# dwcoen1234/longfellow-zk

Hardware: AMD Instinct MI355X
Metric: FFT field-elems/s (batched FFT 2^20 x 1024 rows, Fp128) (higher is better)
Workload: dtype u128 (Fp128 Montgomery, 4 x u32 limbs); 1 GPU; batched FFT 2^20 points x 1024 rows per GPU, Fp128 fftb, in place in HBM; field=Fp128 p=2^128-2^108+1, rows_per_gpu=1024, n=1048576, parallelism=rows sharded x1

## Files before the change

longfellow-zk_amd/csrc/fft.hip:

```cpp
#include <string>
#include <type_traits>

#include "ctx.h"
#include "fp_tile_arith.h"

int lf_lch14_fft_bitsliced(lfgpu_ctx* c, int k, int inverse, size_t rows, unsigned l, u64 coset, void* d_B, size_t ld);

#define TILE_ELTS 8192u

struct TilePlan {
  const elt_t* src;
  elt_t* dst;
  long long src_row, dst_row;
  long long src_tile, dst_tile;
  long long sk, sc, dk, dc;
  u32 logT, logC, nbatch;
  u32 kfast_src, kfast_dst;
  u32 wlds;
};

__device__ __forceinline__ u32 bitrev(u32 x, u32 bits) { return bits ? (__brev(x) >> (32 - bits)) : 0; }

__device__ __forceinline__ u32 lds_slot(u32 k, u32 c, u32 logT, u32 logC) {
  u32 slot = (k << logC) + c;
  if (logT >= 8 && logC >= 3) slot ^= (k >> (logT - 4)) & 15u;
  return slot;
}

struct Fp128Ops {
  static constexpr const char* kKey = "fp";
  static LF_HD elt_t add(elt_t a, elt_t b) { return fp_add(a, b); }
  static LF_HD elt_t sub(elt_t a, elt_t b) { return fp_sub(a, b); }
  static LF_HD elt_t mul_tw(elt_t a, elt_t w) { return fp_mul(a, w); }
  static elt_t hmul(elt_t a, elt_t b) { return fp_mul(a, b); }
  static elt_t one() { return h_fp_of_scalar(1); }
  static elt_t inv(elt_t a) { return h_fp_inv(a); }
};
static u64 h_f64_pow(u64 x, u64 e) {
  u64 r = 0xFFFFFFFFull;
  for (; e; e >>= 1) {
    if (e & 1) r = f64_mul(r, x);
    x = f64_mul(x, x);
  }
  return r;
}
template <bool REAL>
struct F64x2Ops {
  static constexpr const char* kKey = "f64x2";
  static LF_HD elt_t add(elt_t a, elt_t b) { return f64x2_add(a, b); }
  static LF_HD elt_t sub(elt_t a, elt_t b) { return f64x2_sub(a, b); }
  static LF_HD elt_t mul_tw(elt_t a, elt_t w) { return REAL ? f64x2_mul_real(a, w.lo) : f64x2_mul(a, w); }
  static elt_t hmul(elt_t a, elt_t b) { return f64x2_mul(a, b); }
  static elt_t one() { return elt_t{0xFFFFFFFFull, 0ull}; }
  static elt_t inv(elt_t a) {
    const u64 d = f64_add(f64_mul(a.lo, a.lo), f64_mul(a.hi, a.hi));
    return f64x2_mul_real(elt_t{a.lo, f64_sub(0, a.hi)}, h_f64_pow(d, F64_P - 2));
  }
};

template <class O, int R, int FFT_THREADS>
__device__ __forceinline__ void fp_radix_round(elt_t* s, const elt_t* Wl, u32 wsh, u32 logT, u32 logC, u32 st, u32 tid) {
  constexpr u32 N = 1u << R;
  const u32 T = 1u << logT, C = 1u << logC, m = 1u << st;
  for (u32 e = tid; e < (T >> R) * C; e += FFT_THREADS) {
    const u32 c = e & (C - 1), b = e >> logC;
    const u32 j = b & (m - 1);
    const u32 i0 = ((b >> st) << (st + R)) + j;
    elt_t x[N];
    u32 q[N];
#pragma unroll
    for (u32 a = 0; a < N; ++a) {
      q[a] = lds_slot(i0 + a * m, c, logT, logC);
      x[a] = ld16(&s[q[a]]);
    }
#pragma unroll
    for (u32 t = 0; t < (u32)R; ++t) {
      const u32 half = 1u << t;
#pragma unroll
      for (u32 a = 0; a < N; ++a) {
        if (a & half) continue;
        const u32 jj = j + (a & (half - 1)) * m;
        if (t > 0 || j) {
          if ((a & (half - 1)) || j) x[a + half] = O::mul_tw(x[a + half], ld16(&Wl[(size_t)(jj << (logT - 1 - st - t)) << wsh]));
        }
        const elt_t u = x[a], v = x[a + half];
        x[a] = O::add(u, v);
        x[a + half] = O::sub(u, v);
      }
    }
#pragma unroll
    for (u32 a = 0; a < N; ++a) st16(&s[q[a]], x[a]);
  }
}

template <class O, int FFT_THREADS, bool WLDS>
__global__ __launch_bounds__(FFT_THREADS) void fp_fft_tile(TilePlan p, const elt_t* __restrict__ W, u32 wshift,
                                                           const elt_t* __restrict__ tw_lo,
                                                           const elt_t* __restrict__ tw_hi, u32 row_fast) {
  extern __shared__ elt_t s[];
  const u32 T = 1u << p.logT, C = 1u << p.logC, tid = threadIdx.x;
  const u32 bx = row_fast ? blockIdx.y : blockIdx.x, by = row_fast ? blockIdx.x : blockIdx.y;
  const u32 cbase = bx << p.logC;
  const elt_t* src = p.src + (long long)by * p.src_row + (long long)bx * p.src_tile;
  elt_t* dst = p.dst + (long long)by * p.dst_row + (long long)bx * p.dst_tile;

  for (u32 e = tid; e < T * C; e += FFT_THREADS) {
    u32 k, c;
    if (p.kfast_src) { k = e & (T - 1); c = e >> p.logT; } else { c = e & (C - 1); k = e >> p.logC; }
    elt_t v = elt_zero();
    if (cbase + c < p.nbatch) v = ld16(src + (long long)k * p.sk + (long long)c * p.sc);
    st16(&s[lds_slot(bitrev(k, p.logT), c, p.logT, p.logC)], v);
  }
  elt_t* const wl = s + (T << p.logC);
  if (WLDS)
    for (u32 i = tid; i < (T >> 1); i += FFT_THREADS) st16(&wl[i], ld16(&W[(size_t)i << wshift]));
  const u32 wsh = WLDS ? 0 : wshift;
  __syncthreads();
  u32 st = 0;
  while (st < p.logT) {
    const u32 rem = p.logT - st;
    const u32 R = (rem == 3 || rem > 4) ? 3 : (rem >= 2 ? 2 : 1);
    if (WLDS) {
      if (R == 3) fp_radix_round<O, 3, FFT_THREADS>(s, wl, wsh, p.logT, p.logC, st, tid);
      else if (R == 2) fp_radix_round<O, 2, FFT_THREADS>(s, wl, wsh, p.logT, p.logC, st, tid);
      else fp_radix_round<O, 1, FFT_THREADS>(s, wl, wsh, p.logT, p.logC, st, tid);
    } else {
      if (R == 3) fp_radix_round<O, 3, FFT_THREADS>(s, W, wsh, p.logT, p.logC, st, tid);
      else if (R == 2) fp_radix_round<O, 2, FFT_THREADS>(s, W, wsh, p.logT, p.logC, st, tid);
      else fp_radix_round<O, 1, FFT_THREADS>(s, W, wsh, p.logT, p.logC, st, tid);
    }
    __syncthreads();
    st += R;
  }
  for (u32 e = tid; e < T * C; e += FFT_THREADS) {
    u32 j, c;
    if (p.kfast_dst) { j = e & (T - 1); c = e >> p.logT; } else { c = e & (C - 1); j = e >> p.logC; }
    if (cbase + c >= p.nbatch) continue;
    elt_t v = ld16(&s[lds_slot(j, c, p.logT, p.logC)]);
    if (tw_lo) {
      const u32 col = cbase + c, ex = j * col;
      if (ex) {
        if (tw_hi) {
          elt_t t = ld16(&tw_lo[ex & 1023]);
          if (ex >> 10) t = O::mul_tw(t, ld16(&tw_hi[ex >> 10]));
          v = O::mul_tw(v, t);
        } else {
          v = O::mul_tw(v, ld16(&tw_lo[(size_t)j * p.nbatch + col]));
        }
      }
    }
    st16(dst + (long long)j * p.dk + (long long)c * p.dc, v);
  }
}

template <class O>
struct T4Ops : O {
  static __device__ __forceinline__ elt_t add_lazy(elt_t a, elt_t b) { return O::add(a, b); }
  static __device__ __forceinline__ elt_t canon(elt_t a) { return a; }
};
#if defined(__HIP_DEVICE_COMPILE__)
template <>
struct T4Ops<Fp128Ops> : Fp128Ops {
  static __device__ __forceinline__ elt_t add(elt_t a, elt_t b) { return fpt_add(a, b); }
  static __device__ __forceinline__ elt_t add_lazy(elt_t a, elt_t b) { return fpt_add_lazy(a, b); }
  static __device__ __forceinline__ elt_t canon(elt_t a) { return fpt_canon(a); }
  static __device__ __forceinline__ elt_t sub(elt_t a, elt_t b) { return fpt_sub(a, b); }
  static __device__ __forceinline__ elt_t mul_tw(elt_t a, elt_t w) { return fpt_mul(a, w); }
};
#endif

__device__ __forceinline__ u32 t4_slot(u32 p, u32 c, u32 p7) { return ((p << 2) | c) ^ p7; }
__device__ __forceinline__ u32 t4_wslot(u32 i) { return i ^ ((i >> 4) & 15u); }

enum : u32 { T4_CANON = 0, T4_LAZY = 1, T4_LAZY_OUT = 2 };
template <class O, u32 ST, u32 R, bool ROUND0, u32 LZ = T4_CANON>
__device__ __forceinline__ void t4_stages(elt_t* x, u32 j, const elt_t* wl, const elt_t* __restrict__ W, u32 wshift) {
#pragma unroll
  for (u32 t = 0; t < R; ++t) {
    const u32 half = 1u << t;
#pragma unroll
    for (u32 a = 0; a < (1u << R); ++a) {
      if (a & half) continue;
      const u32 jj = j + (a & (half - 1)) * (1u << ST), sh = 9 - ST - t;
      if (!ROUND0) x[a + half] = T4Ops<O>::mul_tw(x[a + half], ld16(&wl[t4_wslot(jj << sh)]));
      else if (a & (half - 1)) x[a + half] = T4Ops<O>::mul_tw(x[a + half], ld16(&W[(size_t)(jj << sh) << wshift]));
      const bool last = LZ == T4_LAZY_OUT && t == R - 1;
      const bool full = LZ == T4_CANON || last || (ROUND0 && ((t == 0 && a != 0) || (t == 1 && a == 4)));
      const elt_t u = last ? T4Ops<O>::canon(x[a]) : x[a], v = x[a + half];
      x[a] = full ? T4Ops<O>::add(u, v) : T4Ops<O>::add_lazy(u, v);
      x[a + half] = T4Ops<O>::sub(u, v);
    }
  }
}

template <class O, u32 LZ>
__device__ __forceinline__ void t4_round0(elt_t* s, const elt_t* y, u32 kb, u32 c, const elt_t* wl, const elt_t* __restrict__ W, u32 wshift) {
  elt_t x[8];
#pragma unroll
  for (u32 a = 0; a < 8; ++a) x[a] = y[((a & 1) << 2) | (a & 2) | (a >> 2)];
  t4_stages<O, 0, 3, true, LZ>(x, 0, wl, W, wshift);
  const u32 b = __brev(kb) >> 25, s0 = t4_slot(8 * b, c, b >> 4), s1 = t4_slot(8 * b + 1, c, b >> 4);
#pragma unroll
  for (u32 a = 0; a < 8; a += 2) {
    st16(&s[s0 + 4 * a], x[a]);
    st16(&s[s1 + 4 * a], x[a + 1]);
  }
}
template <class O, u32 LZ>
__device__ __forceinline__ void t4_round1(elt_t* s, u32 tid, const elt_t* wl, const elt_t* __restrict__ W, u32 wshift) {
  const u32 c = tid & 3, j = (tid >> 2) & 7, h = tid >> 5;
  const u32 s0 = t4_slot(64 * h + j, c, h >> 1);
  elt_t x[8];
#pragma unroll
  for (u32 a = 0; a < 8; ++a) x[a] = ld16(&s[s0 + 32 * a]);
  t4_stages<O, 3, 3, false, LZ>(x, j, wl, W, wshift);
#pragma unroll
  for (u32 a = 0; a < 8; ++a) st16(&s[s0 + 32 * a], x[a]);
}
__device__ __forceinline__ u32 t4_round2_load(elt_t* x, const elt_t* s, u32 e) {
  const u32 c = e & 3, h = e >> 8, j = (e >> 2) & 63;
  const u32 s0 = t4_slot(256 * h + j, c, 2 * h);
#pragma unroll
  for (u32 a = 0; a < 4; ++a) x[a] = ld16(&s[(s0 ^ (a >> 1)) + 256 * a]);
  return s0;
}
template <class O, u32 LZ>
__device__ __forceinline__ void t4_round2_finish(elt_t* s, elt_t* x, u32 e, u32 s0, const elt_t* wl, const elt_t* __restrict__ W, u32 wshift) {
  t4_stages<O, 6, 2, false, LZ>(x, (e >> 2) & 63, wl, W, wshift);
#pragma unroll
  for (u32 a = 0; a < 4; ++a) st16(&s[(s0 ^ (a >> 1)) + 256 * a], x[a]);
}
template <class O, u32 LZ>
__device__ __forceinline__ void t4_round2(elt_t* s, u32 e, const elt_t* wl, const elt_t* __restrict__ W, u32 wshift) {
  elt_t x[4];
  const u32 s0 = t4_round2_load(x, s, e);
  t4_round2_finish<O, LZ>(s, x, e, s0, wl, W, wshift);
}
__device__ __forceinline__ void t4_round3_load(elt_t* x, const elt_t* s, u32 e) {
  const u32 c = e & 3, j = e >> 2;
  const u32 s0 = t4_slot(j, c, j >> 7);
#pragma unroll
  for (u32 a = 0; a < 4; ++a) x[a] = ld16(&s[(s0 ^ (2 * a)) + 1024 * a]);
}

__device__ __forceinline__ void t4_xcd_order(u32 ncb, u32 w, u32& bx, u32& part) {
  if ((ncb & 7) == 0) {
    const u32 per = ncb >> 3, i = w >> 3;
    bx = (w & 7) * per + i % per;
    part = i / per;
  } else {
    bx = w % ncb;
    part = w / ncb;
  }
}
__device__ __forceinline__ void t4a_tw_load(elt_t (*t)[4], const elt_t* __restrict__ tw, u32 nbatch, u32 cbase, u32 tid) {
#pragma unroll
  for (u32 g = 0; g < 2; ++g) {
    const u32 e = tid + 512 * g;
#pragma unroll
    for (u32 a = 0; a < 4; ++a) t[g][a] = ld16(&tw[(size_t)((e >> 2) + 256 * a) * nbatch + cbase + (e & 3)]);
  }
}

template <class O, bool KFAST_SRC, bool TW>
__global__ __launch_bounds__(512, 4) void fp_fft_tile_1024x4(TilePlan p, const elt_t* __restrict__ W, u32 wshift,
                                                             const elt_t* __restrict__ tw, u32 row_fast) {
  extern __shared__ elt_t s[];
  elt_t* const wl = s + 4096;
  const u32 tid = threadIdx.x;
  const u32 bx = row_fast ? blockIdx.y : blockIdx.x, by = row_fast ? blockIdx.x : blockIdx.y;
  {
    const u32 c = KFAST_SRC ? tid >> 7 : tid & 3, kb = KFAST_SRC ? tid & 127 : tid >> 2;
    const elt_t* src = p.src + (long long)by * p.src_row + (long long)bx * p.src_tile + (long long)kb * p.sk + (long long)c * p.sc;
    elt_t y[8];
#pragma unroll
    for (u32 a = 0; a < 8; ++a) y[a] = ld16(src + (long long)(128 * a) * p.sk);
    const elt_t wv = ld16(&W[(size_t)tid << wshift]);
    __builtin_amdgcn_sched_barrier(0);
    t4_round0<O, T4_CANON>(s, y, kb, c, wl, W, wshift);
    st16(&wl[t4_wslot(tid)], wv);
  }
  __syncthreads();
  t4_round1<O, T4_CANON>(s, tid, wl, W, wshift);
  __syncthreads();
  elt_t t[2][4];
  {
    elt_t x[2][4];
    u32 s0[2];
#pragma unroll
    for (u32 g = 0; g < 2; ++g) s0[g] = t4_round2_load(x[g], s, tid + 512 * g);
    if (TW) {
      t4a_tw_load(t, tw, p.nbatch, bx << 2, tid);
      __builtin_amdgcn_sched_barrier(0);
    }
#pragma unroll
    for (u32 g = 0; g < 2; ++g) t4_round2_finish<O, T4_CANON>(s, x[g], tid + 512 * g, s0[g], wl, W, wshift);
  }
  __syncthreads();
  {
    elt_t* dst = p.dst + (long long)by * p.dst_row + (long long)bx * p.dst_tile;
#pragma unroll
    for (u32 g = 0; g < 2; ++g) {
      const u32 e = tid + 512 * g, c = e & 3, j = e >> 2;
      elt_t x[4];
      t4_round3_load(x, s, e);
      t4_stages<O, 8, 2, false>(x, j, wl, W, wshift);
#pragma unroll
      for (u32 a = 0; a < 4; ++a) {
        if (TW) x[a] = T4Ops<O>::mul_tw(x[a], t[g][a]);
        st16(dst + (long long)(j + 256 * a) * p.dk + (long long)c * p.dc, x[a]);
      }
    }
  }
}

__device__ __forceinline__ void t4a_load(elt_t* y, const TilePlan& p, u32 by, u32 bx, u32 tid) {
  const elt_t* src = p.src + (long long)by * p.src_row + (long long)bx * p.src_tile;
  const u32 sk = (u32)p.sk, off = (tid >> 2) * sk + (tid & 3) * (u32)p.sc;
#pragma unroll
  for (u32 a = 0; a < 8; ++a) y[a] = ld16(src + (off + 128 * a * sk));
}

template <class O>
__global__ __launch_bounds__(512, 4) void fp_fft_tile_1024x4_persist(TilePlan p, const elt_t* __restrict__ W, u32 wshift,
                                                                     const elt_t* __restrict__ tw, u32 rows, u32 parts) {
  extern __shared__ elt_t s[];
  elt_t* const wl = s + 4096;
  const u32 tid = threadIdx.x;
  u32 bx, part;
  t4_xcd_order(p.nbatch >> 2, blockIdx.x, bx, part);
  const u32 r0 = (u32)((u64)part * rows / parts), r1 = (u32)((u64)(part + 1) * rows / parts);
  elt_t y[8], t[2][4];
  t4a_tw_load(t, tw, p.nbatch, bx << 2, tid);
  st16(&wl[t4_wslot(tid)], ld16(&W[(size_t)tid << wshift]));
  for (u32 by = r0; by < r1; ++by) {
    u32 lt = tid;
    asm volatile("" : "+v"(lt));
    t4a_load(y, p, by, bx, lt);
    __builtin_amdgcn_sched_barrier(0);
    t4_round0<O, T4_CANON>(s, y, lt >> 2, lt & 3, wl, W, wshift);
    __syncthreads();
    t4_round1<O, T4_CANON>(s, lt, wl, W, wshift);
    __syncthreads();
#pragma unroll
    for (u32 g = 0; g < 2; ++g) t4_round2<O, T4_CANON>(s, lt + 512 * g, wl, W, wshift);
    __syncthreads();
    __builtin_amdgcn_sched_barrier(0);
    {
      elt_t x[2][4];
#pragma unroll
      for (u32 g = 0; g < 2; ++g) t4_round3_load(x[g], s, lt + 512 * g);
      __syncthreads();
      elt_t* dst = p.dst + (long long)by * p.dst_row + (long long)bx * p.dst_tile;
      const u32 dk = (u32)p.dk, dc = (u32)p.dc;
#pragma unroll
      for (u32 g = 0; g < 2; ++g) {
        const u32 e = lt + 512 * g, c = e & 3, j = e >> 2;
        t4_stages<O, 8, 2, false>(x[g], j, wl, W, wshift);
#pragma unroll
        for (u32 a = 0; a < 4; ++a) st16(dst + ((j + 256 * a) * dk + c * dc), T4Ops<O>::mul_tw(x[g][a], t[g][a]));
      }
    }
  }
}

template <class O, bool KFAST_SRC, bool LAZY>
__device__ __forceinline__ void fp_fft_tile_1024x4_tws_body(const TilePlan& p, const elt_t* __restrict__ W, u32 wshift,
                                                            const elt_t* __restrict__ tw, u32 row_fast) {
  constexpr u32 LZ = LAZY ? T4_LAZY : T4_CANON, LZ_OUT = !LAZY ? T4_CANON : KFAST_SRC ? T4_LAZY_OUT : T4_LAZY;
  extern __shared__ elt_t s[];
  elt_t* const wl = s + 4096;
  const u32 tid = threadIdx.x;
  u32 bx, by;
  if (KFAST_SRC) {
    bx = row_fast ? blockIdx.y : blockIdx.x;
    by = row_fast ? blockIdx.x : blockIdx.y;
  } else {
    t4_xcd_order(p.nbatch >> 2, blockIdx.x, bx, by);
  }
  {
    const u32 c = KFAST_SRC ? tid >> 7 : tid & 3, kb = KFAST_SRC ? tid & 127 : tid >> 2;
    const elt_t* src = p.src + (long long)by * p.src_row + (long long)bx * p.src_tile;
    const u32 sk = (u32)p.sk, off = kb * sk + c * (u32)p.sc;
    elt_t y[8], t[8];
#pragma unroll
    for (u32 a = 0; a < 8; ++a) y[a] = ld16(src + (off + 128 * a * sk));
    if (KFAST_SRC) {
      const elt_t* twt = tw + ((size_t)bx << 12);
      const u32 toff = (c << 10) + kb;
#pragma unroll
      for (u32 a = 0; a < 8; ++a) t[a] = ld16(twt + (toff + 128 * a));
    }
    const elt_t wv = ld16(&W[(size_t)tid << wshift]);
    __builtin_amdgcn_sched_barrier(0);
    if (KFAST_SRC) {
#pragma unroll
      for (u32 a = 0; a < 8; ++a) y[a] = T4Ops<O>::mul_tw(y[a], t[a]);
    }
    t4_round0<O, LZ>(s, y, kb, c, wl, W, wshift);
    st16(&wl[t4_wslot(tid)], wv);
  }
  __syncthreads();
  t4_round1<O, LZ>(s, tid, wl, W, wshift);
  __syncthreads();
#pragma unroll
  for (u32 g = 0; g < 2; ++g) t4_round2<O, LZ>(s, tid + 512 * g, wl, W, wshift);
  __syncthreads();
  {
    elt_t* dst = p.dst + (long long)by * p.dst_row + (long long)bx * p.dst_tile;
    const u32 dk = (u32)p.dk, dc = (u32)p.dc;
#pragma unroll
    for (u32 g = 0; g < 2; ++g) {
      const u32 e = tid + 512 * g, c = e & 3, j = e >> 2;
      elt_t x[4];
      t4_round3_load(x, s, e);
      t4_stages<O, 8, 2, false, LZ_OUT>(x, j, wl, W, wshift);
#pragma unroll
      for (u32 a = 0; a < 4; ++a) st16(dst + ((j + 256 * a) * dk + c * dc), x[a]);
    }
  }
}

template <class O, bool KFAST_SRC>
__global__ __launch_bounds__(512, 4) void fp_fft_tile_1024x4_tws(TilePlan p, const elt_t* __restrict__ W, u32 wshift,
                                                                 const elt_t* __restrict__ tw, u32 row_fast) {
  fp_fft_tile_1024x4_tws_body<O, KFAST_SRC, true>(p, W, wshift, tw, row_fast);
}
template <class O, bool KFAST_SRC>
__global__ __launch_bounds__(512, 4) void fp_fft_tile_1024x4_tws_canon(TilePlan p, const elt_t* __restrict__ W, u32 wshift,
                                                                       const elt_t* __restrict__ tw, u32 row_fast) {
  fp_fft_tile_1024x4_tws_body<O, KFAST_SRC, false>(p, W, wshift, tw, row_fast);
}

struct LchTables {
  const elt_t* tbl;
  const elt_t* base;
  u32 nb;
  u32 off[16];
};

template <int FFT_THREADS>
__global__ __launch_bounds__(FFT_THREADS) void lch_fft_tile(TilePlan p, int inverse, LchTables t) {
  extern __shared__ elt_t s[];
  const u32 T = 1u << p.logT, C = 1u << p.logC, tid = threadIdx.x;
  const u32 cbase = blockIdx.x << p.logC;
  const elt_t* src = p.src + (long long)blockIdx.y * p.src_row + (long long)blockIdx.x * p.src_tile;
  elt_t* dst = p.dst + (long long)blockIdx.y * p.dst_row + (long long)blockIdx.x * p.dst_tile;

  for (u32 e = tid; e < T * C; e += FFT_THREADS) {
    u32 k, c;
    if (p.kfast_src) { k = e & (T - 1); c = e >> p.logT; } else { c = e & (C - 1); k = e >> p.logC; }
    elt_t v = elt_zero();
    if (cbase + c < p.nbatch) v = ld16(src + (long long)k * p.sk + (long long)c * p.sc);
    st16(&s[(k << p.logC) + c], v);
  }
  __syncthreads();
  for (u32 step = 0; step < p.logT; ++step) {
    const u32 ii = inverse ? step : (p.logT - 1 - step);
    const u32 sz = 1u << ii;
    for (u32 e = tid; e < (T >> 1) * C; e += FFT_THREADS) {
      u32 c = e & (C - 1), b = e >> p.logC;
      u32 v = b & (sz - 1), u = b >> ii;
      u32 i0 = (u << (ii + 1)) + v, i1 = i0 + sz;
      elt_t tw = ld16(&t.tbl[t.off[ii] + u]);
      if (t.base) {
        u32 cb = cbase + c;
        if (cb >= t.nb) cb = 0;
        tw = gf_add(tw, ld16(&t.base[ii * t.nb + cb]));
      }
      elt_t b0 = ld16(&s[(i0 << p.logC) + c]);
      elt_t b1 = ld16(&s[(i1 << p.logC) + c]);
      if (!inverse) {
        b0 = gf_add(b0, gf_mul(tw, b1));
        b1 = gf_add(b1, b0);
      } else {
        b1 = gf_add(b1, b0);
        b0 = gf_add(b0, gf_mul(tw, b1));
      }
      st16(&s[(i0 << p.logC) + c], b0);
      st16(&s[(i1 << p.logC) + c], b1);
    }
    __syncthreads();
  }
  for (u32 e = tid; e < T * C; e += FFT_THREADS) {
    u32 j, c;
    if (p.kfast_dst) { j = e & (T - 1); c = e >> p.logT; } else { c = e & (C - 1); j = e >> p.logC; }
    if (cbase + c >= p.nbatch) continue;
    st16(dst + (long long)j * p.dk + (long long)c * p.dc, ld16(&s[(j << p.logC) + c]));
  }
}

template <class O>
static int set_lds_limit_fp(lfgpu_ctx* c) {
  LF_HIP(c, hipFuncSetAttribute((const void*)fp_fft_tile<O, 1024, true>, hipFuncAttributeMaxDynamicSharedMemorySize, 160 * 1024));
  LF_HIP(c, hipFuncSetAttribute((const void*)fp_fft_tile<O, 1024, false>, hipFuncAttributeMaxDynamicSharedMemorySize, 160 * 1024));
  LF_HIP(c, hipFuncSetAttribute((const void*)fp_fft_tile<O, 512, true>, hipFuncAttributeMaxDynamicSharedMemorySize, 160 * 1024));
  LF_HIP(c, hipFuncSetAttribute((const void*)fp_fft_tile<O, 512, false>, hipFuncAttributeMaxDynamicSharedMemorySize, 160 * 1024));
  return LFGPU_OK;
}
static int set_lds_limit(lfgpu_ctx* c) {
  if (!(c->attr_done & 1u)) {
    if (const char* e = getenv("LFGPU_TILE_LOG")) {
      int v = atoi(e);
      if (v == 12 || v == 13) c->tile_log = v;
    }
    LF_TRY(set_lds_limit_fp<Fp128Ops>(c));
    const void* const t4[] = {(const void*)fp_fft_tile_1024x4<Fp128Ops, false, true>,
                              (const void*)fp_fft_tile_1024x4<Fp128Ops, true, false>,
                              (const void*)fp_fft_tile_1024x4_persist<Fp128Ops>,
                              (const void*)fp_fft_tile_1024x4_tws<Fp128Ops, false>,
                              (const void*)fp_fft_tile_1024x4_tws<Fp128Ops, true>,
                              (const void*)fp_fft_tile_1024x4_tws_canon<Fp128Ops, false>,
                              (const void*)fp_fft_tile_1024x4_tws_canon<Fp128Ops, true>};
    for (const void* k : t4) LF_HIP(c, hipFuncSetAttribute(k, hipFuncAttributeMaxDynamicSharedMemorySize, 160 * 1024));
    LF_TRY(set_lds_limit_fp<F64x2Ops<true>>(c));
    LF_TRY(set_lds_limit_fp<F64x2Ops<false>>(c));
    LF_HIP(c, hipFuncSetAttribute((const void*)lch_fft_tile<1024>, hipFuncAttributeMaxDynamicSharedMemorySize, TILE_ELTS * 16));
    LF_HIP(c, hipFuncSetAttribute((const void*)lch_fft_tile<512>, hipFuncAttributeMaxDynamicSharedMemorySize, TILE_ELTS * 16));
    c->attr_done |= 1u;
  }
  return LFGPU_OK;
}

static size_t fp_lds_bytes(TilePlan& p) {
  const size_t tile = ((size_t)16 << p.logT) << p.logC, tw = (size_t)8 << p.logT;
  p.wlds = tile + tw <= 160u * 1024u ? 1u : 0u;
  return p.wlds ? tile + tw : tile;
}
template <class O, class... Args>
static void launch_fp(lfgpu_ctx* c, dim3 grid, size_t lds, const TilePlan& p, Args... args) {
  if (c->tile_log == 13) {
    if (p.wlds) hipLaunchKernelGGL((fp_fft_tile<O, 1024, true>), grid, dim3(1024), lds, c->stream, p, args...);
    else hipLaunchKernelGGL((fp_fft_tile<O, 1024, false>), grid, dim3(1024), lds, c->stream, p, args...);
  } else {
    if (p.wlds) hipLaunchKernelGGL((fp_fft_tile<O, 512, true>), grid, dim3(512), lds, c->stream, p, args...);
    else hipLaunchKernelGGL((fp_fft_tile<O, 512, false>), grid, dim3(512), lds, c->stream, p, args...);
  }
}
struct FpSwitches {
  bool tile1024;
  int persist;
  int twside;
  bool other_plan;
  bool lazy;
  bool two_level;
  bool row_fast;
};
static const FpSwitches& fp_switches() {
  static const FpSwitches sw = [] {
    const auto num = [](const char* name, int dflt) { return getenv(name) ? atoi(getenv(name)) : dflt; };
    FpSwitches w;
    w.tile1024 = num("LFGPU_FP_TILE1024", 1) != 0;
    w.persist = num("LFGPU_FP_PERSIST", 1);
    w.twside = num("LFGPU_FP_TWSIDE", 1);
    w.other_plan = getenv("LFGPU_FP_PERSIST") || getenv("LFGPU_FP_TILE1024");
    w.lazy = num("LFGPU_FP_LAZY", 1) != 0;
    w.two_level = num("LFGPU_FP_TW", 0) == 2;
    w.row_fast = num("LFGPU_FP_ROWFAST", 1) != 0;
    return w;
  }();
  return sw;
}
static bool tile_1024x4_fits(const TilePlan& p, bool kfast_src, bool offsets32) {
  if (p.logT != 10 || p.logC != 2 || !p.wlds || p.kfast_src != (kfast_src ? 1u : 0u) || p.kfast_dst != 0 || (p.nbatch & 3) != 0) return false;
  return !offsets32 || (p.sk >= 0 && p.sc >= 0 && p.dk >= 0 && p.dc >= 0 && (u64)p.sk * 1024 + (u64)p.sc * 4 <= 0xffffffffu &&
                        (u64)p.dk * 1024 + (u64)p.dc * 4 <= 0xffffffffu);
}
template <class O>
static bool launch_tile_1024x4_persist(lfgpu_ctx* c, u32 rows, size_t lds, const TilePlan& p, const elt_t* W, u32 wshift, const elt_t* tw) {
  const int mode = fp_switches().persist;
  const u32 ncb = p.nbatch >> 2;
  u32 parts = rows;
  if (mode <= 0 || !tile_1024x4_fits(p, false, true)) return false;
  if (mode >= 2) {
    static const int per_cu = [lds] {
      int n = 0;
      if (hipOccupancyMaxActiveBlocksPerMultiprocessor(&n, (const void*)fp_fft_tile_1024x4_persist<O>, 512, lds) != hipSuccess)
        n = 0;
      return n < 1 ? 1 : n;
    }();
    const u32 fill = (u32)per_cu * (u32)c->num_cu;
    parts = fill / ncb;
    if (parts < 1) parts = 1;
    if (parts > rows) parts = rows;
  }
  if ((u64)ncb * parts > 0x7fffffffu) return false;
  const dim3 grid(ncb * parts);
  hipLaunchKernelGGL((fp_fft_tile_1024x4_persist<O>), grid, dim3(512), lds, c->stream, p, W, wshift, tw, rows, parts);
  return true;
}
template <class O, bool KFAST_SRC, bool TW>
static bool launch_tile_1024x4(lfgpu_ctx* c, dim3 grid, size_t lds, const TilePlan& p, const elt_t* W, u32 wshift, const elt_t* tw,
                               u32 row_fast) {
  if constexpr (std::is_same<O, Fp128Ops>::value) {
    if (fp_switches().tile1024 && c->tile_log == 12 && tile_1024x4_fits(p, KFAST_SRC, false)) {
      if constexpr (!KFAST_SRC && TW)
        if (launch_tile_1024x4_persist<O>(c, row_fast ? grid.x : grid.y, lds, p, W, wshift, tw)) return true;
      hipLaunchKernelGGL((fp_fft_tile_1024x4<O, KFAST_SRC, TW>), grid, dim3(512), lds, c->stream, p, W, wshift, tw, row_fast);
      return true;
    }
  }
  return false;
}
template <class O>
static int fp_twside_mode(const lfgpu_ctx* c, u32 logn1, size_t rows, bool two_level) {
  const int mode = fp_switches().other_plan ? 0 : fp_switches().twside;
  if (!std::is_same<O, Fp128Ops>::value || two_level || c->tile_log != 12 || logn1 != 10 || rows > (0x7fffffffu >> 8)) return 0;
  return mode < 0 ? 0 : mode;
}
template <class O, bool KFAST_SRC>
static bool launch_tile_1024x4_tws(lfgpu_ctx* c, u32 rows, size_t lds, const TilePlan& p, const elt_t* W, u32 wshift, const elt_t* tw,
                                   u32 row_fast) {
  if constexpr (std::is_same<O, Fp128Ops>::value) {
    const u32 ncb = p.nbatch >> 2;
    if (!tile_1024x4_fits(p, KFAST_SRC, true) || (u64)ncb * rows > 0x7fffffffu) return false;
    if (KFAST_SRC && (p.sk != 1 || p.sc != 1024 || p.src_tile != 4096)) return false;
    if (KFAST_SRC && (row_fast ? ncb : rows) > 65535) row_fast = !row_fast;
    const dim3 grid = !KFAST_SRC ? dim3(ncb * rows) : row_fast ? dim3(rows, ncb) : dim3(ncb, rows);
    if (fp_switches().lazy) hipLaunchKernelGGL((fp_fft_tile_1024x4_tws<O, KFAST_SRC>), grid, dim3(512), lds, c->stream, p, W, wshift, tw, row_fast);
    else hipLaunchKernelGGL((fp_fft_tile_1024x4_tws_canon<O, KFAST_SRC>), grid, dim3(512), lds, c->stream, p, W, wshift, tw, row_fast);
    return true;
  }
  return false;
}
template <class... Args>
static void launch_lch(lfgpu_ctx* c, dim3 grid, size_t lds, Args... args) {
  if (c->tile_log == 13)
    hipLaunchKernelGGL(lch_fft_tile<1024>, grid, dim3(1024), lds, c->stream, args...);
  else
    hipLaunchKernelGGL(lch_fft_tile<512>, grid, dim3(512), lds, c->stream, args...);
}

template <class O>
static elt_t fp_reroot(elt_t w, u64 n, u64 r) {
  while (r < n) {
    w = O::hmul(w, w);
    r += r;
  }
  return w;
}

static std::string keyf(const char* fmt, ...) {
  char buf[256];
  va_list ap;
  va_start(ap, fmt);
  vsnprintf(buf, sizeof(buf), fmt, ap);
  va_end(ap);
  return std::string(buf);
}

static TilePlan plan_single(const lfgpu_ctx* c, void* A, size_t rows, u32 logn, size_t ld) {
  TilePlan p{};
  u32 logC = (u32)c->tile_log - logn;
  u32 need = lf_log2(rows);
  if (logC > need) logC = need;
  p.src = (const elt_t*)A;
  p.dst = (elt_t*)A;
  p.src_row = p.dst_row = 0;
  p.src_tile = p.dst_tile = (long long)ld << logC;
  p.sk = p.dk = 1;
  p.sc = p.dc = (long long)ld;
  p.logT = logn;
  p.logC = logC;
  p.nbatch = (u32)rows;
  p.kfast_src = p.kfast_dst = 1;
  return p;
}

template <class O>
static int fp_root_table(lfgpu_ctx* c, const elt_t wn, u32 logn, u32 logTw, std::string* key_out, void** dW) {
  const size_t n = (size_t)1 << logn;
  std::string key = keyf("%sW:%llx:%llx:%u:%u", O::kKey, (u64)wn.lo, (u64)wn.hi, logn, logTw);
  if (!lf_table_lookup(c, key, dW)) {
    std::vector<elt_t> W((size_t)1 << (logTw ? logTw - 1 : 0));
    elt_t wt = fp_reroot<O>(wn, n, (u64)1 << logTw), x = O::one();
    for (size_t i = 0; i < W.size(); ++i) {
      W[i] = x;
      x = O::hmul(x, wt);
    }
    LF_TRY(lf_table(c, key, W.data(), W.size() * 16, dW));
  }
  *key_out = key;
  return LFGPU_OK;
}
template <class O>
static int fp_two_level_tables(lfgpu_ctx* c, const elt_t wn, u32 logn, const std::string& key, void** dlo, void** dhi) {
  std::string klo = key + ":lo", khi = key + ":hi";
  if (!lf_table_lookup(c, klo, dlo) || !lf_table_lookup(c, khi, dhi)) {
    std::vector<elt_t> lo(1024), hi((size_t)1 << (logn > 10 ? logn - 10 : 0));
    elt_t x = O::one();
    for (size_t i = 0; i < 1024; ++i) {
      lo[i] = x;
      x = O::hmul(x, wn);
    }
    elt_t w1024 = x;
    x = O::one();
    for (size_t i = 0; i < hi.size(); ++i) {
      hi[i] = x;
      x = O::hmul(x, w1024);
    }
    LF_TRY(lf_table(c, klo, lo.data(), lo.size() * 16, dlo));
    LF_TRY(lf_table(c, khi, hi.data(), hi.size() * 16, dhi));
  }
  return LFGPU_OK;
}

template <class O>
static int fp_fft_two_pass(lfgpu_ctx* c, const elt_t wn, u32 logn, size_t rows, const elt_t* src, size_t sld, elt_t* dst, long long drow,
                           long long dstep) {
  const size_t n = (size_t)1 << logn;
  const u32 logn2 = 10, logn1 = logn - logn2;
  const u32 logTw = logn1 > logn2 ? logn1 : logn2;
  void *dW = nullptr, *dlo = nullptr, *dhi = nullptr;
  std::string key;
  LF_TRY(fp_root_table<O>(c, wn, logn, logTw, &key, &dW));
  const bool two_level = fp_switches().two_level;
  const size_t n1 = (size_t)1 << logn1, n2 = (size_t)1 << logn2;
  if (two_level) {
    LF_TRY(fp_two_level_tables<O>(c, wn, logn, key, &dlo, &dhi));
  } else {
    std::string kfull = key + ":full";
    if (!lf_table_lookup(c, kfull, &dlo)) {
      std::vector<elt_t> full(n1 * n2);
      elt_t wj = O::one();
      for (size_t j = 0; j < n1; ++j) {
        elt_t x = O::one();
        elt_t* row = &full[j * n2];
        for (size_t k = 0; k < n2; ++k) {
          row[k] = x;
          x = O::hmul(x, wj);
        }
        wj = O::hmul(wj, wn);
      }
      LF_TRY(lf_table(c, kfull, full.data(), full.size() * 16, &dlo));
    }
    dhi = nullptr;
  }
  void* scratch = nullptr;
  LF_TRY(lf_scratch(c, rows * n * 16, &scratch));
  const int twside = fp_twside_mode<O>(c, logn1, rows, two_level);
  {
    TilePlan p{};
    p.logT = logn1;
    p.logC = (u32)c->tile_log - logn1;
    if (p.logC > logn2) p.logC = logn2;
    p.src = src;
    p.dst = (elt_t*)scratch;
    p.src_row = (long long)sld;
    p.dst_row = (long long)n;
    p.src_tile = p.dst_tile = 1ll << p.logC;
    p.sk = p.dk = (long long)n2;
    p.sc = p.dc = 1;
    p.nbatch = (u32)n2;
    p.kfast_src = p.kfast_dst = 0;
    size_t lds = fp_lds_bytes(p);
    const u32 row_fast = (!two_level && rows <= 65535 && fp_switches().row_fast) ? 1u : 0u;
    const dim3 grid = row_fast ? dim3((u32)rows, (u32)(n2 >> p.logC)) : dim3((u32)(n2 >> p.logC), (u32)rows);
    if (twside) {
      if (!launch_tile_1024x4_tws<O, false>(c, (u32)rows, lds, p, (const elt_t*)dW, logTw - logn1, (const elt_t*)nullptr, 0u))
        return lf_fail(c, LFGPU_ERR_UNSUPPORTED, "fp_fft: pass A does not fit the 1024 x 4 tile");
    } else if (two_level || !launch_tile_1024x4<O, false, true>(c, grid, lds, p, (const elt_t*)dW, logTw - logn1, (const elt_t*)dlo, row_fast))
      launch_fp<O>(c, grid, lds, p, (const elt_t*)dW, logTw - logn1, (const elt_t*)dlo, (const elt_t*)dhi, row_fast);
    LF_HIP(c, hipGetLastError());
  }
  {
    TilePlan p{};
    p.logT = logn2;
    p.logC = (u32)c->tile_log - logn2;
    if (p.logC > logn1) p.logC = logn1;
    p.src = (const elt_t*)scratch;
    p.dst = dst;
    p.src_row = (long long)n;
    p.dst_row = drow;
// ... 237 lines not shown
```

longfellow-zk_amd/csrc/fp_tile_arith.h:

```cpp
#pragma once
#include "fields.h"

#if defined(__HIP_DEVICE_COMPILE__)
__device__ __forceinline__ elt_t fpt_add(elt_t a, elt_t b) {
  FP_W(a, a0, a1, a2, a3);
  FP_W(b, b0, b1, b2, b3);
  u32 s0, s1, s2, s3, d0, d1, d2, d3;
  u64 c;
  asm("v_add_co_u32 %0, vcc, %9, %13\n\t"
      "s_nop 1\n\t"
      "v_addc_co_u32 %1, vcc, %10, %14, vcc\n\t"
      "s_nop 1\n\t"
      "v_addc_co_u32 %2, vcc, %11, %15, vcc\n\t"
      "s_nop 1\n\t"
      "v_addc_co_u32 %3, %8, %12, %16, vcc\n\t"
      "v_subrev_co_u32 %4, vcc, 1, %0\n\t"
      "s_nop 1\n\t"
      "v_subbrev_co_u32 %5, vcc, 0, %1, vcc\n\t"
      "s_nop 1\n\t"
      "v_subbrev_co_u32 %6, vcc, 0, %2, vcc\n\t"
      "s_nop 1\n\t"
      "v_subb_co_u32 %7, vcc, %3, %17, vcc\n\t"
      "s_nop 1\n\t"
      "s_andn2_b64 vcc, vcc, %8\n\t"
      "v_cndmask_b32 %4, %4, %0, vcc\n\t"
      "v_cndmask_b32 %5, %5, %1, vcc\n\t"
      "v_cndmask_b32 %6, %6, %2, vcc\n\t"
      "v_cndmask_b32 %7, %7, %3, vcc"
      : "=&v"(s0), "=&v"(s1), "=&v"(s2), "=&v"(s3), "=&v"(d0), "=&v"(d1), "=&v"(d2), "=&v"(d3), "=&s"(c)
      : "v"(a0), "v"(a1), "v"(a2), "v"(a3), "v"(b0), "v"(b1), "v"(b2), "v"(b3), "v"(0xfffff000u)
      : "vcc", "scc");
  return FP_PACK(d0, d1, d2, d3);
}

__device__ __forceinline__ elt_t fpt_add_lazy(elt_t a, elt_t b) {
  FP_W(a, a0, a1, a2, a3);
  FP_W(b, b0, b1, b2, b3);
  u32 d0, d1, d2, d3, e3;
  u64 c;
  asm("v_add_co_u32 %0, vcc, %6, %10\n\t"
      "s_nop 1\n\t"
      "v_addc_co_u32 %1, vcc, %7, %11, vcc\n\t"
      "s_nop 1\n\t"
      "v_addc_co_u32 %2, vcc, %8, %12, vcc\n\t"
      "s_nop 1\n\t"
      "v_addc_co_u32 %3, %5, %9, %13, vcc\n\t"
      "s_nop 1\n\t"
      "v_cndmask_b32 %4, 0, %14, %5\n\t"
      "v_subbrev_co_u32 %0, vcc, 0, %0, %5\n\t"
      "s_nop 1\n\t"
      "v_subbrev_co_u32 %1, vcc, 0, %1, vcc\n\t"
      "s_nop 1\n\t"
      "v_subbrev_co_u32 %2, vcc, 0, %2, vcc\n\t"
      "s_nop 1\n\t"
      "v_subb_co_u32 %3, vcc, %3, %4, vcc"
      : "=&v"(d0), "=&v"(d1), "=&v"(d2), "=&v"(d3), "=&v"(e3), "=&s"(c)
      : "v"(a0), "v"(a1), "v"(a2), "v"(a3), "v"(b0), "v"(b1), "v"(b2), "v"(b3), "v"(0xfffff000u)
      : "vcc");
  return FP_PACK(d0, d1, d2, d3);
}

__device__ __forceinline__ elt_t fpt_canon(elt_t a) {
  FP_W(a, a0, a1, a2, a3);
  u32 d0, d1, d2, d3;
  asm("v_subrev_co_u32 %0, vcc, 1, %4\n\t"
      "s_nop 1\n\t"
      "v_subbrev_co_u32 %1, vcc, 0, %5, vcc\n\t"
      "s_nop 1\n\t"
      "v_subbrev_co_u32 %2, vcc, 0, %6, vcc\n\t"
      "s_nop 1\n\t"
      "v_subb_co_u32 %3, vcc, %7, %8, vcc\n\t"
      "s_nop 1\n\t"
      "v_cndmask_b32 %0, %0, %4, vcc\n\t"
      "v_cndmask_b32 %1, %1, %5, vcc\n\t"
      "v_cndmask_b32 %2, %2, %6, vcc\n\t"
      "v_cndmask_b32 %3, %3, %7, vcc"
      : "=&v"(d0), "=&v"(d1), "=&v"(d2), "=&v"(d3)
      : "v"(a0), "v"(a1), "v"(a2), "v"(a3), "v"(0xfffff000u)
      : "vcc");
  return FP_PACK(d0, d1, d2, d3);
}

__device__ __forceinline__ elt_t fpt_sub(elt_t a, elt_t b) {
  FP_W(a, a0, a1, a2, a3);
  FP_W(b, b0, b1, b2, b3);
  u32 d0, d1, d2, d3, e3;
  u64 bw;
  asm("v_sub_co_u32 %0, vcc, %6, %10\n\t"
      "s_nop 1\n\t"
      "v_subb_co_u32 %1, vcc, %7, %11, vcc\n\t"
      "s_nop 1\n\t"
      "v_subb_co_u32 %2, vcc, %8, %12, vcc\n\t"
      "s_nop 1\n\t"
      "v_subb_co_u32 %3, %5, %9, %13, vcc\n\t"
      "s_nop 1\n\t"
      "v_cndmask_b32 %4, 0, %14, %5\n\t"
      "v_addc_co_u32 %0, vcc, 0, %0, %5\n\t"
      "s_nop 1\n\t"
      "v_addc_co_u32 %1, vcc, 0, %1, vcc\n\t"
      "s_nop 1\n\t"
      "v_addc_co_u32 %2, vcc, 0, %2, vcc\n\t"
      "s_nop 1\n\t"
      "v_addc_co_u32 %3, vcc, %4, %3, vcc"
      : "=&v"(d0), "=&v"(d1), "=&v"(d2), "=&v"(d3), "=&v"(e3), "=&s"(bw)
      : "v"(a0), "v"(a1), "v"(a2), "v"(a3), "v"(b0), "v"(b1), "v"(b2), "v"(b3), "v"(0xfffff000u)
      : "vcc");
  return FP_PACK(d0, d1, d2, d3);
}

#define FPT_MADW(acc, ov, x, y) \
  asm("v_mad_u64_u32 %0, vcc, %2, %3, %0\n\ts_nop 1\n\tv_addc_co_u32 %1, vcc, 0, 0, vcc" : "+v"(acc), "=v"(ov) : "v"(x), "v"(y) : "vcc")
#define FPT_COL(tk, acc, ov) \
  tk = (u32)(acc);           \
  acc = ((acc) >> 32) | ((u64)(ov) << 32)

__device__ __forceinline__ elt_t fpt_mul(elt_t a, elt_t b) {
  FP_W(a, a0, a1, a2, a3);
  FP_W(b, b0, b1, b2, b3);
  u32 t0, t1, t2, t3, t4, t5, t6, t7, ov;
  u64 acc0, acc;
  asm("v_mad_u64_u32 %0, vcc, %1, %2, 0" : "=v"(acc0) : "v"(a0), "v"(b0) : "vcc");
  t0 = (u32)acc0;
  asm("v_mad_u64_u32 %0, vcc, %1, %2, %3" : "=v"(acc) : "v"(a0), "v"(b1), "v"(acc0 >> 32) : "vcc");
  FPT_MADW(acc, ov, a1, b0);
  FPT_COL(t1, acc, ov);
  FP_MAD(acc, a0, b2);
  FPT_MADW(acc, ov, a1, b1);
  FP_MADC(acc, ov, a2, b0);
  FPT_COL(t2, acc, ov);
  FP_MAD(acc, a0, b3);
  FPT_MADW(acc, ov, a1, b2);
  FP_MADC(acc, ov, a2, b1);
  FP_MADC(acc, ov, a3, b0);
  FPT_COL(t3, acc, ov);
  FP_MAD(acc, a1, b3);
  FPT_MADW(acc, ov, a2, b2);
  FP_MADC(acc, ov, a3, b1);
  FPT_COL(t4, acc, ov);
  FP_MAD(acc, a2, b3);
  FPT_MADW(acc, ov, a3, b2);
  FPT_COL(t5, acc, ov);
  FP_MAD(acc, a3, b3);
  t6 = (u32)acc;
  t7 = (u32)(acc >> 32);
  const u32 k = t0 << 12;
  u32 d0, d1, d2, d3;
  {
    u32 e3;
    u64 cy, b;
    asm("v_add_co_u32 %7, %9, %7, %11\n\t"
        "v_sub_co_u32 %0, vcc, %13, %4\n\t"
        "s_nop 1\n\t"
        "v_subb_co_u32 %1, vcc, %14, %5, vcc\n\t"
        "s_nop 1\n\t"
        "v_subb_co_u32 %2, vcc, %15, %6, vcc\n\t"
        "s_nop 1\n\t"
        "v_subb_co_u32 %3, %10, %16, %7, vcc\n\t"
        "v_alignbit_b32 %4, %5, %4, 20\n\t"
        "v_alignbit_b32 %5, %6, %5, 20\n\t"
        "v_alignbit_b32 %6, %7, %6, 20\n\t"
        "v_lshrrev_b32 %7, 20, %7\n\t"
        "v_addc_co_u32 %0, vcc, %0, %4, %9\n\t"
        "s_nop 1\n\t"
        "v_addc_co_u32 %1, vcc, %1, %5, vcc\n\t"
        "s_nop 1\n\t"
        "v_addc_co_u32 %2, vcc, %2, %6, vcc\n\t"
        "s_nop 1\n\t"
        "v_addc_co_u32 %3, %9, %3, %7, vcc\n\t"
        "s_nop 1\n\t"
        "s_andn2_b64 %9, %10, %9\n\t"
        "v_cndmask_b32 %8, 0, %12, %9\n\t"
        "v_addc_co_u32 %0, vcc, 0, %0, %9\n\t"
        "s_nop 1\n\t"
        "v_addc_co_u32 %1, vcc, 0, %1, vcc\n\t"
        "s_nop 1\n\t"
        "v_addc_co_u32 %2, vcc, 0, %2, vcc\n\t"
        "s_nop 1\n\t"
        "v_addc_co_u32 %3, vcc, %8, %3, vcc"
        : "=&v"(d0), "=&v"(d1), "=&v"(d2), "=&v"(d3), "+v"(t0), "+v"(t1), "+v"(t2), "+v"(t3), "=&v"(e3), "=&s"(cy), "=&s"(b)
        : "v"(k), "v"(0xfffff000u), "v"(t4), "v"(t5), "v"(t6), "v"(t7)
        : "vcc", "scc");
  }
  return FP_PACK(d0, d1, d2, d3);
}
#else
LF_HD elt_t fpt_add(elt_t a, elt_t b) { return fp_add_c(a, b); }
LF_HD elt_t fpt_sub(elt_t a, elt_t b) { return fp_sub_c(a, b); }
LF_HD elt_t fpt_canon(elt_t a) { return fp_canon128(a); }
LF_HD elt_t fpt_add_lazy(elt_t a, elt_t b) {
  const u64 lo = a.lo + b.lo, c0 = lo < a.lo, h0 = a.hi + b.hi, hi = h0 + c0;
  if (!((h0 < a.hi) | (hi < c0))) return elt_t{lo, hi};
  return elt_t{lo - FP_P_LO, hi - FP_P_HI - (lo < FP_P_LO)};
}
LF_HD elt_t fpt_mul(elt_t a, elt_t b) { return fp_mul_c(fp_canon128(a), b); }
#endif
```

Baseline: 47.47 billion field-elems/s.

## Add radix-8 round-1 FFT tile kernel with wave-uniform SGPR twiddles

```diff
diff --git a/longfellow-zk_amd/csrc/fft.hip b/longfellow-zk_amd/csrc/fft.hip
--- a/longfellow-zk_amd/csrc/fft.hip
+++ b/longfellow-zk_amd/csrc/fft.hip
@@ -157,6 +157,7 @@
 struct T4Ops : O {
   static __device__ __forceinline__ elt_t add_lazy(elt_t a, elt_t b) { return O::add(a, b); }
   static __device__ __forceinline__ elt_t canon(elt_t a) { return a; }
+  static __device__ __forceinline__ elt_t mul_tw_sw(elt_t a, elt_t w) { return O::mul_tw(a, w); }
 };
 #if defined(__HIP_DEVICE_COMPILE__)
 template <>
@@ -166,6 +167,7 @@
   static __device__ __forceinline__ elt_t canon(elt_t a) { return fpt_canon(a); }
   static __device__ __forceinline__ elt_t sub(elt_t a, elt_t b) { return fpt_sub(a, b); }
   static __device__ __forceinline__ elt_t mul_tw(elt_t a, elt_t w) { return fpt_mul(a, w); }
+  static __device__ __forceinline__ elt_t mul_tw_sw(elt_t a, elt_t w) { return fpt_mul_sw(a, w); }
 };
 #endif
 
@@ -430,6 +432,149 @@
 __global__ __launch_bounds__(512, 4) void fp_fft_tile_1024x4_tws_canon(TilePlan p, const elt_t* __restrict__ W, u32 wshift,
                                                                        const elt_t* __restrict__ tw, u32 row_fast) {
   fp_fft_tile_1024x4_tws_body<O, KFAST_SRC, false>(p, W, wshift, tw, row_fast);
+}
+
+__device__ __forceinline__ u32 t4w_swz(u32 p) { return (p >> 7) ^ ((p >> 4) & 12u); }
+__device__ __forceinline__ u32 t4w_slot(u32 p, u32 c) { return ((p << 2) | c) ^ t4w_swz(p); }
+
+template <u32 ST>
+__device__ __forceinline__ u32 t4w_tw_index(u32 j, u32 m) {
+  const u32 t = m < 1 ? 0 : m < 3 ? 1 : 2, k = m + 1 - (1u << t);
+  return (j + (k << ST)) << (9 - ST - t);
+}
+enum : u32 { T4W_R0 = 0, T4W_R1 = 1, T4W_R1_J0 = 2 };
+template <class O, u32 MODE>
+__device__ __forceinline__ void t4w_stages(elt_t* x, const elt_t* w) {
+#pragma unroll
+  for (u32 t = 0; t < 3; ++t) {
+    const u32 half = 1u << t;
+#pragma unroll
+    for (u32 a = 0; a < 8; ++a) {
+      if (a & half) continue;
+      const u32 k = a & (half - 1);
+      const bool skip = MODE != T4W_R1 && k == 0, full = MODE == T4W_R0 && ((t == 0 && a != 0) || (t == 1 && a == 4));
+      const elt_t u = x[a], v = !skip ? T4Ops<O>::mul_tw_sw(x[a + half], w[half - 1 + k]) : MODE == T4W_R1_J0 ? T4Ops<O>::canon(x[a + half]) : x[a + half];
+      x[a] = full ? T4Ops<O>::add(u, v) : T4Ops<O>::add_lazy(u, v);
+      x[a + half] = T4Ops<O>::sub(u, v);
+    }
+  }
+}
+template <class O>
+__device__ __forceinline__ void t4w_round0(elt_t* s, const elt_t* y, u32 kb, u32 c, const elt_t* w) {
+  elt_t x[8];
+#pragma unroll
+  for (u32 a = 0; a < 8; ++a) x[a] = y[((a & 1) << 2) | (a & 2) | (a >> 2)];
+  t4w_stages<O, T4W_R0>(x, w);
+  const u32 s0 = t4w_slot((__brev(kb) >> 25) << 3, c);
+#pragma unroll
+  for (u32 a = 0; a < 8; ++a) st16(&s[(s0 ^ (4 * (a & 3))) + 16 * (a >> 2)], x[a]);
+}
+template <class O, u32 MODE>
+__device__ __forceinline__ void t4w_round1_wave(elt_t* s, u32 s0, const elt_t* w) {
+  elt_t x[8];
+#pragma unroll
+  for (u32 a = 0; a < 8; ++a) x[a] = ld16(&s[s0 + 32 * a]);
+  t4w_stages<O, MODE>(x, w);
+#pragma unroll
+  for (u32 a = 0; a < 8; ++a) st16(&s[s0 + 32 * a], x[a]);
+}
+template <class O>
+__device__ __forceinline__ void t4w_round1(elt_t* s, u32 tid, u32 j, const elt_t* w) {
+  const u32 c = tid & 3, h = (tid >> 2) & 15;
+  const u32 s0 = t4w_slot(64 * h + j, c);
+  if (j == 0) {
+    asm volatile("; round 1, j = 0");
+    t4w_round1_wave<O, T4W_R1_J0>(s, s0, w);
+    asm volatile("; round 1, j = 0: stored");
+  } else {
+    asm volatile("; round 1, j > 0");
+    t4w_round1_wave<O, T4W_R1>(s, s0, w);
+    asm volatile("; round 1, j > 0: stored");
+  }
+}
+template <class O>
+__device__ __forceinline__ void t4w_round2(elt_t* s, u32 e, const elt_t* wl, const elt_t* __restrict__ W, u32 wshift) {
+  const u32 c = e & 3, h = e >> 8, j = (e >> 2) & 63;
+  const u32 s0 = t4w_slot(256 * h + j, c);
+  elt_t x[4];
+#pragma unroll
+  for (u32 a = 0; a < 4; ++a) x[a] = ld16(&s[(s0 ^ t4w_swz(64 * a)) + 256 * a]);
+  t4_stages<O, 6, 2, false, T4_LAZY>(x, j, wl, W, wshift);
+#pragma unroll
+  for (u32 a = 0; a < 4; ++a) st16(&s[(s0 ^ t4w_swz(64 * a)) + 256 * a], x[a]);
+}
+__device__ __forceinline__ void t4w_round3_load(elt_t* x, const elt_t* s, u32 e) {
+  const u32 s0 = t4w_slot(e >> 2, e & 3);
+#pragma unroll
+  for (u32 a = 0; a < 4; ++a) x[a] = ld16(&s[(s0 ^ (2 * a)) + 1024 * a]);
+}
+
+template <class O, bool KFAST_SRC>
+__global__ __launch_bounds__(512, 4) void fp_fft_tile_1024x4_tw2(TilePlan p, const elt_t* __restrict__ W, u32 wshift,
+                                                                 const elt_t* __restrict__ tw, u32 row_fast) {
+  extern __shared__ elt_t s[];
+  elt_t* const wl = s + 4096;
+  const u32 tid = threadIdx.x, j1 = __builtin_amdgcn_readfirstlane(tid >> 6);
+  u32 bx, by;
+  if (KFAST_SRC) {
+    bx = row_fast ? blockIdx.y : blockIdx.x;
+    by = row_fast ? blockIdx.x : blockIdx.y;
+  } else {
+    t4_xcd_order(p.nbatch >> 2, blockIdx.x, bx, by);
+  }
+  elt_t w0[7] = {}, w1[7];
+  {
+    const u32 c = KFAST_SRC ? tid >> 7 : tid & 3, kb = KFAST_SRC ? tid & 127 : tid >> 2;
+    const elt_t* src = p.src + (long long)by * p.src_row + (long long)bx * p.src_tile;
+    const u32 sk = (u32)p.sk, off = kb * sk + c * (u32)p.sc;
+    elt_t y[8], t[8];
+#pragma unroll
+    for (u32 a = 0; a < 8; ++a) y[a] = ld16(src + (off + 128 * a * sk));
+    if (KFAST_SRC) {
+      const elt_t* twt = tw + ((size_t)bx << 12);
+      const u32 toff = (c << 10) + kb;
+#pragma unroll
+      for (u32 a = 0; a < 8; ++a) t[a] = ld16(twt + (toff + 128 * a));
+    }
+    const elt_t wv = ld16(&W[(size_t)tid << wshift]);
+#pragma unroll
+    for (u32 m = 0; m < 7; ++m) {
+      w1[m] = ld16(&W[(size_t)t4w_tw_index<3>(j1, m) << wshift]);
+      if (m >= 4) w0[m] = ld16(&W[(size_t)t4w_tw_index<0>(0, m) << wshift]);
+    }
+#pragma unroll
+    for (u32 m = 0; m < 7; ++m) {
+      asm volatile("" : "+s"(w1[m].lo), "+s"(w1[m].hi));
+      if (m >= 4) asm volatile("" : "+s"(w0[m].lo), "+s"(w0[m].hi));
+    }
+    w0[2] = w0[5];
+    __builtin_amdgcn_sched_barrier(0);
+    if (KFAST_SRC) {
+#pragma unroll
+      for (u32 a = 0; a < 8; ++a) y[a] = T4Ops<O>::mul_tw(y[a], t[a]);
+    }
+    t4w_round0<O>(s, y, kb, c, w0);
+    st16(&wl[t4_wslot(tid)], wv);
+  }
+  __syncthreads();
+  t4w_round1<O>(s, tid, j1, w1);
+  __syncthreads();
+#pragma unroll
+  for (u32 g = 0; g < 2; ++g) t4w_round2<O>(s, tid + 512 * g, wl, W, wshift);
+  __syncthreads();
+  {
+    elt_t* dst = p.dst + (long long)by * p.dst_row + (long long)bx * p.dst_tile;
+    const u32 dk = (u32)p.dk, dc = (u32)p.dc;
+#pragma unroll
+    for (u32 g = 0; g < 2; ++g) {
+      const u32 e = tid + 512 * g, c = e & 3, j = e >> 2;
+      elt_t x[4];
+      t4w_round3_load(x, s, e);
+      t4_stages<O, 8, 2, false, KFAST_SRC ? T4_LAZY_OUT : T4_LAZY>(x, j, wl, W, wshift);
+#pragma unroll
+      for (u32 a = 0; a < 4; ++a) st16(dst + ((j + 256 * a) * dk + c * dc), x[a]);
+    }
+  }
 }
 
 struct LchTables {
@@ -511,7 +656,9 @@
                               (const void*)fp_fft_tile_1024x4_tws<Fp128Ops, false>,
                               (const void*)fp_fft_tile_1024x4_tws<Fp128Ops, true>,
                               (const void*)fp_fft_tile_1024x4_tws_canon<Fp128Ops, false>,
-                              (const void*)fp_fft_tile_1024x4_tws_canon<Fp128Ops, true>};
+                              (const void*)fp_fft_tile_1024x4_tws_canon<Fp128Ops, true>,
+                              (const void*)fp_fft_tile_1024x4_tw2<Fp128Ops, false>,
+                              (const void*)fp_fft_tile_1024x4_tw2<Fp128Ops, true>};
     for (const void* k : t4) LF_HIP(c, hipFuncSetAttribute(k, hipFuncAttributeMaxDynamicSharedMemorySize, 160 * 1024));
     LF_TRY(set_lds_limit_fp<F64x2Ops<true>>(c));
     LF_TRY(set_lds_limit_fp<F64x2Ops<false>>(c));
@@ -543,6 +690,7 @@
   int twside;
   bool other_plan;
   bool lazy;
+  bool r1wave;
   bool two_level;
   bool row_fast;
 };
@@ -555,6 +703,7 @@
     w.twside = num("LFGPU_FP_TWSIDE", 1);
     w.other_plan = getenv("LFGPU_FP_PERSIST") || getenv("LFGPU_FP_TILE1024");
     w.lazy = num("LFGPU_FP_LAZY", 1) != 0;
+    w.r1wave = num("LFGPU_FP_R1WAVE", 1) != 0;
     w.two_level = num("LFGPU_FP_TW", 0) == 2;
     w.row_fast = num("LFGPU_FP_ROWFAST", 1) != 0;
     return w;
@@ -617,8 +766,9 @@
     if (KFAST_SRC && (p.sk != 1 || p.sc != 1024 || p.src_tile != 4096)) return false;
     if (KFAST_SRC && (row_fast ? ncb : rows) > 65535) row_fast = !row_fast;
     const dim3 grid = !KFAST_SRC ? dim3(ncb * rows) : row_fast ? dim3(rows, ncb) : dim3(ncb, rows);
-    if (fp_switches().lazy) hipLaunchKernelGGL((fp_fft_tile_1024x4_tws<O, KFAST_SRC>), grid, dim3(512), lds, c->stream, p, W, wshift, tw, row_fast);
-    else hipLaunchKernelGGL((fp_fft_tile_1024x4_tws_canon<O, KFAST_SRC>), grid, dim3(512), lds, c->stream, p, W, wshift, tw, row_fast);
+    if (!fp_switches().lazy) hipLaunchKernelGGL((fp_fft_tile_1024x4_tws_canon<O, KFAST_SRC>), grid, dim3(512), lds, c->stream, p, W, wshift, tw, row_fast);
+    else if (fp_switches().r1wave) hipLaunchKernelGGL((fp_fft_tile_1024x4_tw2<O, KFAST_SRC>), grid, dim3(512), lds, c->stream, p, W, wshift, tw, row_fast);
+    else hipLaunchKernelGGL((fp_fft_tile_1024x4_tws<O, KFAST_SRC>), grid, dim3(512), lds, c->stream, p, W, wshift, tw, row_fast);
     return true;
   }
   return false;
diff --git a/longfellow-zk_amd/csrc/fp_tile_arith.h b/longfellow-zk_amd/csrc/fp_tile_arith.h
--- a/longfellow-zk_amd/csrc/fp_tile_arith.h
+++ b/longfellow-zk_amd/csrc/fp_tile_arith.h
@@ -108,41 +108,51 @@
   return FP_PACK(d0, d1, d2, d3);
 }
 
-#define FPT_MADW(acc, ov, x, y) \
-  asm("v_mad_u64_u32 %0, vcc, %2, %3, %0\n\ts_nop 1\n\tv_addc_co_u32 %1, vcc, 0, 0, vcc" : "+v"(acc), "=v"(ov) : "v"(x), "v"(y) : "vcc")
+#define FPT_MAD(C, acc, x, y) asm("v_mad_u64_u32 %0, vcc, %1, %2, %0" : "+v"(acc) : "v"(x), C(y) : "vcc")
+#define FPT_MADC(C, acc, ov, x, y) \
+  asm("v_mad_u64_u32 %0, vcc, %2, %3, %0\n\ts_nop 1\n\tv_addc_co_u32 %1, vcc, 0, %1, vcc" : "+v"(acc), "+v"(ov) : "v"(x), C(y) : "vcc")
+#define FPT_MADW(C, acc, ov, x, y) \
+  asm("v_mad_u64_u32 %0, vcc, %2, %3, %0\n\ts_nop 1\n\tv_addc_co_u32 %1, vcc, 0, 0, vcc" : "+v"(acc), "=v"(ov) : "v"(x), C(y) : "vcc")
 #define FPT_COL(tk, acc, ov) \
   tk = (u32)(acc);           \
   acc = ((acc) >> 32) | ((u64)(ov) << 32)
-
-__device__ __forceinline__ elt_t fpt_mul(elt_t a, elt_t b) {
+#define FPT_COLUMNS(C)                                                                                 \
+  asm("v_mad_u64_u32 %0, vcc, %1, %2, 0" : "=v"(acc0) : "v"(a0), C(b0) : "vcc");                       \
+  t0 = (u32)acc0;                                                                                      \
+  asm("v_mad_u64_u32 %0, vcc, %1, %2, %3" : "=v"(acc) : "v"(a0), C(b1), "v"(acc0 >> 32) : "vcc");      \
+  FPT_MADW(C, acc, ov, a1, b0);                                                                        \
+  FPT_COL(t1, acc, ov);                                                                                \
+  FPT_MAD(C, acc, a0, b2);                                                                             \
+  FPT_MADW(C, acc, ov, a1, b1);                                                                        \
+  FPT_MADC(C, acc, ov, a2, b0);                                                                        \
+  FPT_COL(t2, acc, ov);                                                                                \
+  FPT_MAD(C, acc, a0, b3);                                                                             \
+  FPT_MADW(C, acc, ov, a1, b2);                                                                        \
+  FPT_MADC(C, acc, ov, a2, b1);                                                                        \
+  FPT_MADC(C, acc, ov, a3, b0);                                                                        \
+  FPT_COL(t3, acc, ov);                                                                                \
+  FPT_MAD(C, acc, a1, b3);                                                                             \
+  FPT_MADW(C, acc, ov, a2, b2);                                                                        \
+  FPT_MADC(C, acc, ov, a3, b1);                                                                        \
+  FPT_COL(t4, acc, ov);                                                                                \
+  FPT_MAD(C, acc, a2, b3);                                                                             \
+  FPT_MADW(C, acc, ov, a3, b2);                                                                        \
+  FPT_COL(t5, acc, ov);                                                                                \
+  FPT_MAD(C, acc, a3, b3);                                                                             \
+  t6 = (u32)acc;                                                                                       \
+  t7 = (u32)(acc >> 32)
+
+template <bool SW>
+__device__ __forceinline__ elt_t fpt_mul_t(elt_t a, elt_t b) {
   FP_W(a, a0, a1, a2, a3);
   FP_W(b, b0, b1, b2, b3);
   u32 t0, t1, t2, t3, t4, t5, t6, t7, ov;
   u64 acc0, acc;
-  asm("v_mad_u64_u32 %0, vcc, %1, %2, 0" : "=v"(acc0) : "v"(a0), "v"(b0) : "vcc");
-  t0 = (u32)acc0;
-  asm("v_mad_u64_u32 %0, vcc, %1, %2, %3" : "=v"(acc) : "v"(a0), "v"(b1), "v"(acc0 >> 32) : "vcc");
-  FPT_MADW(acc, ov, a1, b0);
-  FPT_COL(t1, acc, ov);
-  FP_MAD(acc, a0, b2);
-  FPT_MADW(acc, ov, a1, b1);
-  FP_MADC(acc, ov, a2, b0);
-  FPT_COL(t2, acc, ov);
-  FP_MAD(acc, a0, b3);
-  FPT_MADW(acc, ov, a1, b2);
-  FP_MADC(acc, ov, a2, b1);
-  FP_MADC(acc, ov, a3, b0);
-  FPT_COL(t3, acc, ov);
-  FP_MAD(acc, a1, b3);
-  FPT_MADW(acc, ov, a2, b2);
-  FP_MADC(acc, ov, a3, b1);
-  FPT_COL(t4, acc, ov);
-  FP_MAD(acc, a2, b3);
-  FPT_MADW(acc, ov, a3, b2);
-  FPT_COL(t5, acc, ov);
-  FP_MAD(acc, a3, b3);
-  t6 = (u32)acc;
-  t7 = (u32)(acc >> 32);
+  if constexpr (SW) {
+    FPT_COLUMNS("s");
+  } else {
+    FPT_COLUMNS("v");
+  }
   const u32 k = t0 << 12;
   u32 d0, d1, d2, d3;
   {
@@ -183,6 +193,8 @@
   }
   return FP_PACK(d0, d1, d2, d3);
 }
+__device__ __forceinline__ elt_t fpt_mul(elt_t a, elt_t b) { return fpt_mul_t<false>(a, b); }
+__device__ __forceinline__ elt_t fpt_mul_sw(elt_t a, elt_t b) { return fpt_mul_t<true>(a, b); }
 #else
 LF_HD elt_t fpt_add(elt_t a, elt_t b) { return fp_add_c(a, b); }
 LF_HD elt_t fpt_sub(elt_t a, elt_t b) { return fp_sub_c(a, b); }
@@ -193,4 +205,5 @@
   return elt_t{lo - FP_P_LO, hi - FP_P_HI - (lo < FP_P_LO)};
 }
 LF_HD elt_t fpt_mul(elt_t a, elt_t b) { return fp_mul_c(fp_canon128(a), b); }
+LF_HD elt_t fpt_mul_sw(elt_t a, elt_t b) { return fpt_mul(a, b); }
 #endif
```

After: 48.15 billion field-elems/s (median of 6 runs). +1.4%, better.
